# renjie-liang/HUAL

Measured on AMD Instinct MI355X. Metric: train clips/sec, higher is better.
Workload: dtype f32 (fp16x3 / bf16x3 split-operand MFMA, fp32 accumulate); 1 GPU; Charades-STA SeqPAN train step (fwd+bwd+clip+AdamWD, dropout 0.2), batch 64/GPU, T=128, vdim=1024, L=20, C=8, dim=128, 8 heads, 2 attention layers, random init; ONE batch resident in HBM, batch assembly (hual_assemble_batch) outside the timed region; global_batch=64, T=128, vdim=1024, L=20, parallelism=dp1, launch=hipGraph, video_dtype=f32

## Files before the change

hual_amd/csrc/api_kernels.cpp:

```cpp
#include "../../include/hual_seqpan.h"
#include "common.h"
#include "gemm.h"
#include "mproj.h"
#include "attn.h"
#include "heads.h"
#include "rowops.h"

namespace hual {
const char* last_error_cstr();
}

using namespace hual;

extern "C" {

int hual_abi_version(void) { return HUAL_ABI_VERSION; }
uint64_t hual_cfg_bytes(void) { return sizeof(hual_cfg); }
const char* hual_last_error(void) { return hual::last_error_cstr(); }

int hual_linear_dw(const float* A, int lda, const float* dY, int ldy, float* dW, int ldw, float* db, int M, int K,
                   int N, int workgroups, void* scratch, uint64_t scratch_bytes, void* stream) {
  HUAL_REQUIRE(A && dY && dW, "hual_linear_dw: null pointer");
  HUAL_REQUIRE(M > 0 && K % 16 == 0 && N == 128, "hual_linear_dw: K % 16 == 0 and N == 128 required");
  HUAL_REQUIRE(workgroups >= 0, "hual_linear_dw: workgroups >= 0 (0: one per CU)");
  HUAL_REQUIRE(scratch && scratch_bytes >= 4 * dw_table_words(1), "hual_linear_dw: scratch table too small");
  DwJob j;
  dw_job_init(j);
  j.npieces = 1;
  j.A[0] = A; j.lda[0] = lda; j.kw[0] = K; j.dW[0] = dW; j.ldw = ldw;
  j.dY = dY; j.ldy = ldy; j.M = M; j.N = N; j.db = db;
  DropCfg d = make_dropcfg(nullptr, 0.f);
  return launch_dw(&j, 1, d, (hipStream_t)stream, reinterpret_cast<DwJob*>(scratch), true, workgroups);
}

int hual_linear_bf16x3(const float* A, int lda, const float* W, int trans_w, const float* bias, float* Y, int ldy, int M,
                       int K, int N, int act, void* scratch, uint64_t scratch_bytes, void* stream) {
  HUAL_REQUIRE(A && W && Y && scratch, "hual_linear_bf16x3: null pointer");
  HUAL_REQUIRE(M > 0 && K > 0 && N > 0 && act >= 0 && act <= 1, "hual_linear_bf16x3: bad shape / act (0 none, 1 relu)");
  HUAL_REQUIRE((lda % 4) == 0 && (ldy % 4) == 0, "hual_linear_bf16x3: leading dims must be multiples of 4");
  const uint32_t off = 0, boff = 0;
  MProjArgs g{};
  g.R = M; g.MT = mproj_rows(M);
  if (!trans_w) {
    HUAL_REQUIRE(N == 128 && K % 8 == 0, "hual_linear_bf16x3: W must be [K,128] with K % 8 == 0");
    HUAL_REQUIRE(scratch_bytes >= (uint64_t)((K + 127) / 128) * 65536, "hual_linear_bf16x3: scratch too small (ceil(K/128) * 65536 bytes)");
// ... 92 lines not shown
```

hual_amd/csrc/dablock.h:

```cpp
#pragma once
#include "common.h"
#include "rowops.h"

namespace hual {

#define HUAL_LNPROJ_MAX 5
struct LnProjArgs {
  const float* x;
  const float* xa; int pre_site; float* x_out;
  uint8_t* pre_bits; uint8_t* y1_bits;
  const float* x2;
  const float* g1; const float* b1; float* y1;
  int drop_site1;
  const float* g2; const float* b2; float* y2;
  float* mean; float* rstd;
  int nproj;
  const float* wimg[HUAL_LNPROJ_MAX];
  const float* bias[HUAL_LNPROJ_MAX];
  float* out[HUAL_LNPROJ_MAX]; int ldo[HUAL_LNPROJ_MAX];
  int src[HUAL_LNPROJ_MAX];
  int accum[HUAL_LNPROJ_MAX];
  int act[HUAL_LNPROJ_MAX];
  int out_site[HUAL_LNPROJ_MAX];
  uint8_t* out_bits[HUAL_LNPROJ_MAX];
// ... 22 lines not shown
  int R; int MT;
  int Nv;
  uint32_t drop_row0;
};
int da_post_rows(int R, int Nv = 0);
int launch_da_post(const DaPostArgs& a, const DropCfg& drop, hipStream_t s, const LnProjArgs* tail = nullptr);

}

namespace hual {

#define HUAL_LNBWD_MAX 6
struct LnProjBwdArgs {
  int nsteps;
  const float* A[HUAL_LNBWD_MAX]; int lda[HUAL_LNBWD_MAX];
  const uint8_t* a_bits[HUAL_LNBWD_MAX];
  float* a_save[HUAL_LNBWD_MAX];
  const float* wimg_t[HUAL_LNBWD_MAX];
  int dst[HUAL_LNBWD_MAX];
  const float* add_dy1;
  const uint8_t* dy1_bits;
  const float* x; const float* mean; const float* rstd;
  const float* g1; const float* g2;
  const float* add1;
  float* dx;
  float* dz; const uint8_t* dz_bits;
  float* part;
  int R; int MT; uint32_t drop_row0;
  int Nv;
  const float* pre_x; const float* pre_mean; const float* pre_rstd; const float* pre_g; const float* pre_dy; const float* pre_add;
// ... 18 lines not shown
```

hual_amd/csrc/dablock.hip:

```cpp
#include "dablock.h"
#include "tilecore.h"
#include "prof.h"

using namespace hual;

__device__ __forceinline__ float row16_max(float v) {
  v = fmaxf(v, dpp_xor_partner(v, 1));
  v = fmaxf(v, dpp_xor_partner(v, 2));
  v = fmaxf(v, dpp_xor_partner(v, 4));
  v = fmaxf(v, dpp_xor_partner(v, 8));
  return v;
}
__device__ __forceinline__ float4 sig4(float4 v) { return make_float4(sigmoidf_(v.x), sigmoidf_(v.y), sigmoidf_(v.z), sigmoidf_(v.w)); }

#include "lnproj_body.h"

template <int NT, bool PLAIN>
__global__ __launch_bounds__(CB_THREADS) void ln_proj_kernel(LnProjArgs a, DropCfg drop) {
  extern __shared__ __attribute__((aligned(16))) char lp_lds[];
  ln_proj_body<NT, false, PLAIN>(a, drop, lp_lds);
}
template <int NT>
__global__ __launch_bounds__(CB_THREADS) void ln_proj_pair_kernel(LnProjArgs a0, LnProjArgs a1, DropCfg drop) {
  extern __shared__ __attribute__((aligned(16))) char lp_lds[];
// ... 301 lines not shown
  if (tile_ < 0) return false;
  const int r0 = tile_ * MT;
  const int RE = min(R, r0 + MT);
  const int j = lane & 15, g = lane >> 4, ecol = 16 * wave + 4 * g;
  const DropRegs dr = drop_load(drop);

  TfW w[2];
  tf_load_w(w[0], a.wimg_t[0], wave, lane);
  float4 nv[LB_U], xv[LB_U], a1v[LB_U];
  float mu[LB_U], rsd[LB_U];
  constexpr bool pre = PRE;
  const float* add1p = pre ? (a.pre_add ? a.pre_add : a.x) : (a.add1 ? a.add1 : a.x);
  const float* a0p = pre ? a.pre_dy : a.A[0];
  const int lda0 = pre ? HUAL_D : a.lda[0];
  uint32_t nkb[LB_U];
  const int nsteps = SIX ? 6 : (MID ? 1 : a.nsteps);
  auto has_bits = [&](int k) { return !SIX && a.a_bits[k] != nullptr; };
  auto to_second = [&](int k) { return SIX ? k >= 4 : a.dst[k] != 0; };
  const bool has_g2 = SIX || (!MID && a.g2 != nullptr), has_add_dy1 = SIX || (!MID && a.add_dy1 != nullptr), has_dy1_bits = !SIX && a.dy1_bits != nullptr;
  const uint8_t* kb0p = has_bits(0) ? a.a_bits[0] : reinterpret_cast<const uint8_t*>(a.x);
  float4 pxv[LB_U];
  float pmu[LB_U], prs[LB_U];
#pragma unroll
  for (int u = 0; u < LB_U; ++u) {
    const int row = min(r0 + grp + 16 * u, R - 1);
    nv[u] = ld4(a0p + (size_t)row * lda0 + col);
    nkb[u] = SIX ? 0u : kb0p[(size_t)row * 16 + (l32 >> 1)];
    xv[u] = ld4(a.x + (size_t)row * HUAL_D + col);
    a1v[u] = ld4(add1p + (size_t)row * HUAL_D + col);
    mu[u] = a.mean[row];
    rsd[u] = a.rstd[row];
    if (pre) { pxv[u] = ld4(a.pre_x + (size_t)row * HUAL_D + col); pmu[u] = a.pre_mean[row]; prs[u] = a.pre_rstd[row]; }
  }
  const float4 g1 = ld4(a.g1 + col);
  float4 sg2 = f4zero(), sb2 = f4zero();
  if (pre) {
    const float4 pg = ld4(a.pre_g + col);
#pragma unroll
    for (int u = 0; u < LB_U; ++u) {
      const int lr = grp + 16 * u;
      const bool ok = lr < MT && r0 + lr < RE;
// ... 13 lines not shown
  }
  const float4 g2 = has_g2 ? ld4(a.g2 + col) : f4zero();
  float4 addt[NT];
  const float* addp = has_add_dy1 ? a.add_dy1 : a.x;
#pragma unroll
  for (int rt = 0; rt < NT; ++rt) addt[rt] = (SIX || MID) ? f4zero() : ld4(addp + (uint32_t)min(r0 + 16 * rt + j, R - 1) * (uint32_t)HUAL_D + (uint32_t)ecol);
  auto fill = [&](int k) {
    char* S = (k & 1) ? S1 : S0;
    float* ai = (k & 1) ? ainv1 : ainv0;
#pragma unroll
    for (int u = 0; u < LB_U; ++u) {
      const int lr = grp + 16 * u, row = r0 + lr;
      if (lr >= MT) continue;
      const bool ok = row < RE;
      float4 v = ok ? nv[u] : f4zero();
      if (has_bits(k)) {
        if (dr.enabled) v = f4_select((nkb[u] >> (4 * (l32 & 1))) & 15u, make_float4(v.x * dr.scale, v.y * dr.scale, v.z * dr.scale, v.w * dr.scale));
        if (ok && a.a_save[k]) st4_nt(a.a_save[k] + (size_t)row * HUAL_D + col, v);
      }
      const float inv = cb_store_operand(S, S + LB_ROWS * 256, lr, l32, v);
      if (l32 == 0) ai[lr] = ok ? inv : 0.f;
    }
  };
  HUAL_STAMP_K(4, 0);
  fill(0);
  HUAL_STAMP_K(4, 1);
  float4 acc0[NT], acc1[NT];
  bool first0 = true, first1 = true;
#pragma unroll
  for (int rt = 0; rt < NT; ++rt) { acc0[rt] = f4zero(); acc1[rt] = f4zero(); }
#pragma unroll
  for (int k = 0; k < HUAL_LNBWD_MAX; ++k) {
    if (k >= nsteps) break;
    const bool more = k + 1 < nsteps;
    if (SIX && k == 5) {
#pragma unroll
      for (int rt = 0; rt < NT; ++rt) addt[rt] = ld4(addp + (uint32_t)min(r0 + 16 * rt + j, R - 1) * (uint32_t)HUAL_D + (uint32_t)ecol);
    }
    if (more) {
      const uint8_t* nbp = has_bits(k + 1) ? a.a_bits[k + 1] : reinterpret_cast<const uint8_t*>(a.x);
      const float* nap = a.A[k + 1];
      const int nld = a.lda[k + 1];
#pragma unroll
      for (int u = 0; u < LB_U; ++u) {
        const size_t row = (size_t)min(r0 + grp + 16 * u, R - 1);
        nv[u] = ld4(nap + row * nld + col);
        nkb[u] = SIX ? 0u : nbp[row * 16 + (l32 >> 1)];
      }
      tf_load_w(w[(k + 1) & 1], a.wimg_t[k + 1], wave, lane);
    }
// ... 452 lines not shown
    return 0;
  }
  switch (cdiv(a.MT, 16)) {
    case 1: { HUAL_DYN_LDS(da_post_kernel<1>, 160 * 1024); HUAL_LAUNCH(flops, bytes, da_post_kernel<1>, grid, dim3(CB_THREADS), lds, s, a, drop); break; }
    case 2: { HUAL_DYN_LDS(da_post_kernel<2>, 160 * 1024); HUAL_LAUNCH(flops, bytes, da_post_kernel<2>, grid, dim3(CB_THREADS), lds, s, a, drop); break; }
    default: { HUAL_DYN_LDS(da_post_kernel<3>, 160 * 1024); HUAL_LAUNCH(flops, bytes, da_post_kernel<3>, grid, dim3(CB_THREADS), lds, s, a, drop); break; }
  }
  HUAL_CHECK_HIP(hipGetLastError());
  return 0;
}

int ln_proj_bwd_rows(int R, int Nv) { return tile_rows(R, Nv, LB_ROWS); }
int ln_proj_bwd_blocks(int R, int Nv) { return cdiv(R, ln_proj_bwd_rows(R, Nv)); }

static bool ln_proj_bwd_six(const LnProjBwdArgs& a) {
  if (a.pre_x || a.nsteps != 6 || !a.g2 || !a.add_dy1 || a.dy1_bits || !a.add1) return false;
  for (int k = 0; k < 6; ++k)
    if (a.a_bits[k] || a.a_save[k] || (a.dst[k] != 0) != (k >= 4)) return false;
  return true;
}

static int check_ln_proj_bwd(const LnProjBwdArgs& a) {
  HUAL_REQUIRE(a.nsteps >= 1 && a.nsteps <= HUAL_LNBWD_MAX && a.R > 0, "ln_proj_bwd: step count / rows");
  HUAL_REQUIRE(a.MT >= 1 && a.MT <= LB_ROWS, "ln_proj_bwd: MT must be 1..48");
  HUAL_REQUIRE(a.x && a.mean && a.rstd && a.g1 && a.dx && a.part, "ln_proj_bwd: null tensor");
  bool any1 = false;
  for (int k = 0; k < a.nsteps; ++k) {
    HUAL_REQUIRE((a.A[k] || (k == 0 && a.pre_x)) && a.wimg_t[k] && (a.lda[k] % 4) == 0, "ln_proj_bwd: product operand");
    HUAL_REQUIRE(a.dst[k] == 0 || a.g2, "ln_proj_bwd: product for the absent second layer norm");
    any1 = any1 || a.dst[k] != 0;
  }
  HUAL_REQUIRE(!a.g2 || any1, "ln_proj_bwd: second layer norm without a product");
  HUAL_REQUIRE(!a.pre_x || (!a.g2 && !a.add1 && a.pre_mean && a.pre_rstd && a.pre_g && a.pre_dy), "ln_proj_bwd: layer-norm prologue");
  return 0;
}
static void ln_proj_bwd_work(const LnProjBwdArgs& a, double& flops, double& bytes) {
  const double rows = (double)a.R;
  flops += 2.0 * rows * HUAL_D * HUAL_D * a.nsteps;
  bytes += 4.0 * (rows * HUAL_D * ((a.pre_x ? 7.0 : 4.0) + a.nsteps) + (double)a.nsteps * HUAL_D * HUAL_D);
}

int launch_ln_proj_bwd(const LnProjBwdArgs& a, const DropCfg& drop, hipStream_t s) {
  int rc = check_ln_proj_bwd(a);
  if (rc) return rc;
  const size_t lds = LB_LDS;
  double flops = 0.0, bytes = 0.0;
  ln_proj_bwd_work(a, flops, bytes);
  const dim3 grid(xcd_clip_grid(a.R, a.Nv, a.MT));
  const bool six = ln_proj_bwd_six(a);
#define LN_BWD_NT(NT)                                                                                                   \
  {                                                                                                                     \
    if (a.pre_x) { HUAL_DYN_LDS((ln_proj_bwd_kernel<true, NT>), 160 * 1024); HUAL_LAUNCH(flops, bytes, (ln_proj_bwd_kernel<true, NT>), grid, dim3(CB_THREADS), lds, s, a, drop); } \
    else if (six) { HUAL_DYN_LDS((ln_proj_bwd_kernel<false, NT, true>), 160 * 1024); HUAL_LAUNCH(flops, bytes, (ln_proj_bwd_kernel<false, NT, true>), grid, dim3(CB_THREADS), lds, s, a, drop); } \
    else { HUAL_DYN_LDS((ln_proj_bwd_kernel<false, NT>), 160 * 1024); HUAL_LAUNCH(flops, bytes, (ln_proj_bwd_kernel<false, NT>), grid, dim3(CB_THREADS), lds, s, a, drop); }      \
// ... 68 lines not shown
```

hual_amd/csrc/gemm.h:

```cpp
#pragma once
#include "common.h"
#include "embed_args.h"

namespace hual {

#define HUAL_MAX_PIECES 4

struct DwJob {
  const float* A[HUAL_MAX_PIECES];
  const float* A2[HUAL_MAX_PIECES];
  int lda[HUAL_MAX_PIECES];
  int lda2[HUAL_MAX_PIECES];
  int kw[HUAL_MAX_PIECES];
  int npieces;
  int a_drop_site;
  uint32_t a_drop_row0;
  float* dW[HUAL_MAX_PIECES];
  int ldw;
  const float* dY; int ldy;
  int M, N;
  float* db;
  int a_bf16;
  const uint8_t* a_keep; int ld_keep;
};

#define HUAL_MAX_DW_JOBS 12
struct DwBatch {
  DwJob j[HUAL_MAX_DW_JOBS];
};

#define HUAL_PACK_BLOCK_BYTES (128 * 512)
struct PackExtra {
  const int32_t* lens; const int32_t* word_ids; float* rowmask; float* loss_acc; int B, T, L;
  float* zero_ptr; size_t zero_n;
  const float* E; float lambda; float* dE_ortho;
  int gather_tasks; int gather_rows; EmbedArgs emb; DropCfg drop;
  int wall_K; uint32_t wall_off, wall_boff;
  uint32_t* ovf; int novf;
// ... 30 lines not shown
```

hual_amd/csrc/gemm.hip:

```cpp
#include "gemm.h"
#include <type_traits>
#include "philox.h"
#include "bf16x3.h"
#include "tilecore.h"
#include "prof.h"
#include "ortho.h"
#include "embed_gather.h"
#include <math.h>
#include <stdlib.h>
#include <stdio.h>
#include <string.h>

namespace hual {

void dw_job_init(DwJob& j) {
  ::memset((void*)&j, 0, sizeof(j));
  j.a_drop_site = -1;
}

}

using namespace hual;

__device__ __forceinline__ float4 f4mul(float4 a, float4 b) { return make_float4(a.x * b.x, a.y * b.y, a.z * b.z, a.w * b.w); }
// ... 232 lines not shown
#define DWB_PLAIN 0
#define DWB_PROD 1
#define DWB_DROP 2
template <int MODE, int DEPTH>
__device__ __forceinline__ void dw_f16_segment(const DwJob& job, const int p, const int kb, const int m_lo, const int m_hi,
                                                const DropCfg& drop, char* ldsb, float4 (*bred)[32]) {
  const int lane = threadIdx.x & 63, wave = threadIdx.x >> 6;
  const int i = lane & 31, h = lane >> 5;
  const int kq = wave >> 2, nq = wave & 3;
  const int k0 = kb * 128;
  const int kw = job.kw[p];
  const char* Ap = reinterpret_cast<const char*>(job.A[p]);
  const char* A2p = MODE == DWB_PROD ? reinterpret_cast<const char*>(job.A2[p]) : nullptr;
  const int lda = job.lda[p], lda2 = job.lda2[p];
  const char* Yp = reinterpret_cast<const char*>(job.dY);
  const int ldy = job.ldy;
  constexpr bool PLAIN = MODE == DWB_PLAIN;
  const bool adrop = MODE == DWB_DROP && job.a_drop_site >= 0 && drop.enabled;
  const uint32_t asite = (uint32_t)job.a_drop_site;
  const uint32_t arow0 = job.a_drop_row0;
  const bool dob = (job.db != nullptr) && p == 0 && kb == 0;
  const bool abf = MODE == DWB_DROP && job.a_bf16 != 0;

  f32x16 acc[2];
#pragma unroll
  for (int c = 0; c < 2; ++c)
#pragma unroll
    for (int r = 0; r < 16; ++r) acc[c][r] = 0.f;
  float4 bsum = f4zero();
  float* mxs = reinterpret_cast<float*>(&bred[0][0]);
  float s_y = 0.f, s_y_inv = 0.f;
  float s_a = 0.f, s_a_inv = 0.f;

  const int srow = threadIdx.x >> 5, c4 = threadIdx.x & 31;
  const int kcol = k0 + 4 * c4;
  const bool kin = kcol < kw;
  const uint32_t esz = abf ? 2u : 4u;
  const uint32_t aoff = ((uint32_t)srow * (uint32_t)lda + (uint32_t)kcol) * esz;
  const uint32_t yoff = ((uint32_t)srow * (uint32_t)ldy + 4u * (uint32_t)c4) * 4u;
  struct Stage { float4 a[DWB_RU], y[DWB_RU], a2[MODE == DWB_PROD ? DWB_RU : 1]; uint32_t keep[DWB_RU]; };
  const uint32_t a2off = ((uint32_t)srow * (uint32_t)lda2 + (uint32_t)kcol) * 4u;
  const uint8_t* keepp = MODE == DWB_DROP ? job.a_keep : nullptr;
  const uint32_t koff = (uint32_t)srow * (uint32_t)job.ld_keep + (uint32_t)(kcol >> 3);
  Stage st[DEPTH - 1];
  auto stage_load = [&](int mt, Stage& st) {
    const char* Ab = Ap + (size_t)mt * lda * esz;
    const char* Yb = Yp + (size_t)mt * ldy * 4;
#pragma unroll
    for (int u = 0; u < DWB_RU; ++u) {
      const int m = mt + srow + 16 * u;
      float4 a = f4zero(), y = f4zero();
      if (m < m_hi) {
        if (kin) {
          if (abf) {
            const uint2 raw = ld2_global(Ab + 16u * u * (uint32_t)lda * 2u + aoff);
            a.x = __uint_as_float(raw.x);
            a.y = __uint_as_float(raw.y);
          } else {
            a = ld4_global(Ab + 16u * u * (uint32_t)lda * 4u + aoff);
          }
          if (MODE == DWB_PROD && A2p) st.a2[u] = ld4_global(A2p + (size_t)mt * lda2 * 4 + 16u * u * (uint32_t)lda2 * 4u + a2off);
        }
        y = ld4_global(Yb + 16u * u * (uint32_t)ldy * 4u + yoff);
        if (MODE == DWB_DROP && keepp && kin) st.keep[u] = ld1_global(keepp + (size_t)mt * job.ld_keep + 16u * u * (uint32_t)job.ld_keep + koff);
      }
      st.a[u] = a;
      st.y[u] = y;
    }
  };
  auto stage_store = [&](int buf, int mt, const Stage& st) {
    char* base = ldsb + buf * 4 * DWB_PLANE;
#pragma unroll
    for (int u = 0; u < DWB_RU; ++u) {
      const int row = srow + 16 * u;
      const int off = tile256_off(row, c4 >> 1) + 8 * (c4 & 1);
      float4 a = st.a[u];
      if (!PLAIN) {
        const int m = mt + row;
        const bool live = m < m_hi && kin;
        if (abf) {
          const uint32_t r0 = __float_as_uint(a.x), r1 = __float_as_uint(a.y);
          a = make_float4(__uint_as_float(r0 << 16), __uint_as_float(r0 & 0xffff0000u), __uint_as_float(r1 << 16),
                          __uint_as_float(r1 & 0xffff0000u));
        }
        if (MODE == DWB_PROD && A2p && live) a = f4mul(a, st.a2[u]);
        if (adrop && live) {
          a = f4mul(a, mask_from_bits4((st.keep[u] >> (4 * (c4 & 1))) & 15u, drop.scale));
        }
      }
      uint2 hi, lo;
      f16_split4_s(a, s_a, hi, lo);
      *reinterpret_cast<uint2*>(base + off) = hi;
      *reinterpret_cast<uint2*>(base + DWB_PLANE + off) = lo;
      f16_split4_s(st.y[u], s_y, hi, lo);
      *reinterpret_cast<uint2*>(base + 2 * DWB_PLANE + off) = hi;
      *reinterpret_cast<uint2*>(base + 3 * DWB_PLANE + off) = lo;
      bsum = f4add(bsum, st.y[u]);
    }
  };
  const int gq = (lane >> 2) & 3, gp = lane & 3, ghalf = (lane >> 4) & 1, gh = lane >> 5;
  auto tr_off = [&](int colbase, int ks, int rr) {
    const int row = 16 * ks + 8 * gh + 4 * rr + gq;
    const int ch = ((colbase + 16 * ghalf) >> 3) + (gp >> 1);
    return tile256_off(row, ch) + 8 * (gp & 1);
  };
  auto products = [&](int buf) {
    const char* base = ldsb + buf * 4 * DWB_PLANE;
#pragma unroll
    for (int ks = 0; ks < DWB_TM / 16; ++ks) {
      const int y0 = tr_off(nq * 32, ks, 0), y1 = tr_off(nq * 32, ks, 1);
      const f16x8 yh = join_tr_f16(lds_read_tr16(base + 2 * DWB_PLANE, y0), lds_read_tr16(base + 2 * DWB_PLANE, y1));
      const f16x8 yl = join_tr_f16(lds_read_tr16(base + 3 * DWB_PLANE, y0), lds_read_tr16(base + 3 * DWB_PLANE, y1));
// ... 4 lines not shown
        const f16x8 al = join_tr_f16(lds_read_tr16(base + DWB_PLANE, o0), lds_read_tr16(base + DWB_PLANE, o1));
        acc[c] = __builtin_amdgcn_mfma_f32_32x32x16_f16(ah, yh, acc[c], 0, 0, 0);
        acc[c] = __builtin_amdgcn_mfma_f32_32x32x16_f16(ah, yl, acc[c], 0, 0, 0);
        acc[c] = __builtin_amdgcn_mfma_f32_32x32x16_f16(al, yh, acc[c], 0, 0, 0);
      }
    }
  };

  auto put_max = [&](const Stage& st, int par) {
#ifdef DWB_EXP_FIXSCALE
    return;
#endif
    float m = 0.f, ma = 0.f;
#pragma unroll
    for (int u = 0; u < DWB_RU; ++u) {
      m = fmaxf(m, f4absmax(st.y[u]));
      float4 a = st.a[u];
      if (abf) {
        const uint32_t r0 = __float_as_uint(a.x), r1 = __float_as_uint(a.y);
        a = make_float4(__uint_as_float(r0 << 16), __uint_as_float(r0 & 0xffff0000u), __uint_as_float(r1 << 16), __uint_as_float(r1 & 0xffff0000u));
      }
      if (MODE == DWB_PROD && A2p) a = f4mul(a, st.a2[u]);
      ma = fmaxf(ma, f4absmax(a));
    }
    if (adrop) ma *= drop.scale;
    m = fast_max32(m);
    m = fmaxf(m, lane_xor32_partner(m));
    ma = fast_max32(ma);
    ma = fmaxf(ma, lane_xor32_partner(ma));
    if (lane == 0) { mxs[par * 16 + wave] = m; mxs[par * 16 + 8 + wave] = ma; }
  };
// ... 83 lines not shown
  if (dob) {
    bred[srow][c4] = bsum;
    __syncthreads();
    if (threadIdx.x < 128) {
      const int cc = threadIdx.x;
      float s = 0.f;
#pragma unroll
      for (int k = 0; k < 16; ++k) s += reinterpret_cast<const float*>(&bred[k][cc >> 2])[cc & 3];
      atomic_add_global(job.db + cc, s);
    }
  }
}

__device__ __forceinline__ void dw_f16_any_segment(const DwJob& job, const int p, const int kb, const int m_lo, const int m_hi,
                                                    const DropCfg& drop, char* ldsb, float4 (*bred)[32]) {
  if (job.A2[p]) dw_f16_segment<DWB_PROD, 2>(job, p, kb, m_lo, m_hi, drop, ldsb, bred);
  else if (job.a_bf16 || job.a_drop_site >= 0) dw_f16_segment<DWB_DROP, 4>(job, p, kb, m_lo, m_hi, drop, ldsb, bred);
  else dw_f16_segment<DWB_PLAIN, 4>(job, p, kb, m_lo, m_hi, drop, ldsb, bred);
}

#ifdef HUAL_STAMPS
#define DW_STAMP_SLOTS 16
__device__ unsigned long long g_dw_stamps[2048 * DW_STAMP_SLOTS];
extern "C" int hual_debug_dw_stamps(unsigned long long* out, int n) {
  return (int)hipMemcpyFromSymbol(out, HIP_SYMBOL(g_dw_stamps), sizeof(unsigned long long) * (size_t)n);
}
#define DW_STAMP(i, v) do { if (threadIdx.x == 0 && blockIdx.x < 2048 && (i) < DW_STAMP_SLOTS) g_dw_stamps[blockIdx.x * DW_STAMP_SLOTS + (i)] = (v); } while (0)
#else
#define DW_STAMP(i, v) do { } while (0)
#endif
#define DW_UNIT_COST 72
// ... 37 lines not shown
  DW_STAMP(5, (unsigned long long)j);
  int nseg = 0, nnp = 0;
  while (t < t_end) {
    const DwJob& job = table[j];
    const int per_unit = (job.M + DWB_TM - 1) / DWB_TM;
    const int local = t - prefix[j];
    int unit = local / per_unit;
    const int tile = local - unit * per_unit;
    const int cnt = min(per_unit - tile, t_end - t);
    int p = 0;
    for (p = 0; p < job.npieces; ++p) {
      const int nkb = (job.kw[p] + 127) >> 7;
      if (unit < nkb) break;
      unit -= nkb;
    }
    const bool plain = !job.a_bf16 && !job.A2[p] && job.a_drop_site < 0;
    dw_f16_any_segment(job, p, unit, tile * DWB_TM, min((tile + cnt) * DWB_TM, job.M), drop, reinterpret_cast<char*>(lds), bred);
    t += cnt;
    if (t >= prefix[j + 1]) ++j;
    __syncthreads();
    DW_STAMP(7 + nseg, __builtin_readcyclecounter());
    ++nseg;
    nnp += plain ? 0 : 1;
  }
  DW_STAMP(2, __builtin_readcyclecounter());
  DW_STAMP(4, (unsigned long long)nseg);
  DW_STAMP(6, (unsigned long long)nnp);
}

namespace hual {

// ... 61 lines not shown
  return 0;
}

static int dw_check(const DwJob& j, int& kbs, double& flops, double& bytes) {
  HUAL_REQUIRE(j.M > 0 && j.N == 128, "launch_dw: N must be 128");
  HUAL_REQUIRE(j.npieces >= 1 && j.npieces <= HUAL_MAX_PIECES, "launch_dw: pieces");
  kbs = 0;
  double kt = 0.0;
  for (int p = 0; p < j.npieces; ++p) {
    HUAL_REQUIRE(j.kw[p] > 0 && (j.kw[p] % 16) == 0, "launch_dw: piece width must be a multiple of 16");
    HUAL_REQUIRE(j.A[p] && j.dW[p], "launch_dw: null operand");
    HUAL_REQUIRE((j.lda[p] % 4) == 0 && (j.ldy % 4) == 0, "launch_dw: leading dims must be multiples of 4");
    kbs += cdiv(j.kw[p], 128);
    kt += j.kw[p];
  }
  flops += 2.0 * j.M * kt * j.N;
  bytes += 4.0 * ((double)j.M * kt + (double)j.M * j.N + kt * j.N);
  return 0;
}

int launch_dw(const DwJob* jobs, int n, const DropCfg& drop, hipStream_t stream, DwJob* table, bool write_table, int blocks) {
  HUAL_REQUIRE(table != nullptr && n >= 1, "launch_dw: job table");
  for (int i = 0; i < n; ++i)
    HUAL_REQUIRE(!jobs[i].a_bf16 || (jobs[i].npieces == 1 && !jobs[i].A2[0] && (jobs[i].lda[0] % 4) == 0),
                 "dw: a bfloat16 operand needs one piece, no product prologue");
  double flops = 0.0, bytes = 0.0;
  int tiles = 0, cost = 0;
  static const int wts[3] = {32, 46, 46};
  for (int base = 0; base < n; base += HUAL_MAX_DW_JOBS) {
    const int cnt = n - base < HUAL_MAX_DW_JOBS ? n - base : HUAL_MAX_DW_JOBS;
    DwBatch b;
    DwPlanPart pre;
    for (int i = 0; i < cnt; ++i) {
      const DwJob& jb = jobs[base + i];
      int kbs;
      int rc = dw_check(jb, kbs, flops, bytes);
      if (rc) return rc;
      b.j[i] = jb;
      bool prod = false;
      for (int p = 0; p < jb.npieces; ++p) prod = prod || jb.A2[p] != nullptr;
      const int w = (jb.a_drop_site >= 0 || jb.a_bf16) ? wts[2] : prod ? wts[1] : wts[0];
      pre.tiles[i] = tiles;
      pre.cost[i] = cost;
      pre.w[i] = w;
      tiles += kbs * cdiv(jb.M, DWB_TM);
      cost += kbs * (DW_UNIT_COST + cdiv(jb.M, DWB_TM) * w);
    }
    for (int i = cnt; i <= HUAL_MAX_DW_JOBS; ++i) { pre.tiles[i] = tiles; pre.cost[i] = cost; pre.w[i] = 1; }
    if (write_table) HUAL_LAUNCH(0.0, 0.0, dw_table_write_kernel, dim3(1), dim3(64), 0, stream, b, pre, table, base, cnt, n);
  }
  int dev = 0, cus = 256;
  HUAL_CHECK_HIP(hipGetDevice(&dev));
  HUAL_CHECK_HIP(hipDeviceGetAttribute(&cus, hipDeviceAttributeMultiprocessorCount, dev));
  int nblocks = blocks > 0 ? blocks : cus;
  if (nblocks > tiles) nblocks = tiles;
// ... 8 lines not shown
```

hual_amd/csrc/seqpan.hip:

```cpp
#include "attn.h"
#include "prof.h"
#include "cq.h"
#include "convblock.h"
#include "dablock.h"
#include "embed.h"
#include "gemm.h"
#include "heads.h"
#include "mproj.h"
#include "optim.h"
#include "params.h"
#include "rowops.h"
#include <stdlib.h>
#include <string.h>
#include <algorithm>
#include <unordered_map>
#include <vector>

namespace hual {
const char* last_error_cstr();
}
using namespace hual;

namespace {

// ... 1002 lines not shown
        attn_job_init(a[k]);
        a[k].Q = qkv; a[k].ldq = 3 * D; a[k].B = B; a[k].qmask = rowmask; a[k].kmask = rowmask; a[k].lddo = D; a[k].lddq = D;
        a[k].O = (k & 1) ? x_att : s_att; a[k].ldo = D;
      }
      a[0].K = qkv + D; a[0].V = qkv + 2 * D; a[0].ldkv = 3 * D; a[0].Tq = T; a[0].Tk = T; a[0].qrow0 = 0; a[0].krow0 = 0;
      a[0].dO = d_satt; a[0].dQ = dq_self; a[0].dK = d_qkv + D; a[0].dV = d_qkv + 2 * D; a[0].lddkv = 3 * D; a[0].drop_site = site + 0;
      a[1].K = ktvt; a[1].V = ktvt + D; a[1].ldkv = 2 * D; a[1].Tq = T; a[1].Tk = L; a[1].qrow0 = 0; a[1].krow0 = Nv;
      a[1].dO = d_xatt; a[1].dQ = dq_cross; a[1].dK = d_ktvt; a[1].dV = d_ktvt + D; a[1].lddkv = 2 * D; a[1].drop_site = site + 1;
      a[2].K = qkv + D; a[2].V = qkv + 2 * D; a[2].ldkv = 3 * D; a[2].Tq = L; a[2].Tk = L; a[2].qrow0 = Nv; a[2].krow0 = Nv;
      a[2].dO = d_satt; a[2].dQ = dq_self; a[2].dK = d_qkv + D; a[2].dV = d_qkv + 2 * D; a[2].lddkv = 3 * D; a[2].drop_site = site + 0;
      a[3].K = ktvt; a[3].V = ktvt + D; a[3].ldkv = 2 * D; a[3].Tq = L; a[3].Tk = T; a[3].qrow0 = Nv; a[3].krow0 = 0;
      a[3].dO = d_xatt; a[3].dQ = dq_cross; a[3].dK = d_ktvt; a[3].dV = d_ktvt + D; a[3].lddkv = 2 * D; a[3].drop_site = site + 1;
      for (int k = 0; k < 4; ++k) set_dmask(c, a[k], t + ".dm" + std::to_string(k));
      c.attn_bwd(a, 4);
    }
    c.push_dw(mkdw(ln1, D, D, dq_self, D, R, c.g(d.query.k), c.g(d.query.b)));
    c.push_dw(mkdw(ln1, D, D, dq_cross, D, R, c.g(d.query.k), c.g(d.query.b)));
    c.push_dw(mkdw(ln1, D, D, d_qkv + D, 3 * D, R, c.g(d.f_key.k), c.g(d.f_key.b)));
    c.push_dw(mkdw(ln1, D, D, d_qkv + 2 * D, 3 * D, R, c.g(d.f_value.k), c.g(d.f_value.b)));
    c.push_dw(mkdw(lnt, D, D, d_ktvt, 2 * D, R, c.g(d.t_key.k), c.g(d.t_key.b)));
    c.push_dw(mkdw(lnt, D, D, d_ktvt + D, 2 * D, R, c.g(d.t_value.k), c.g(d.t_value.b)));
    float* d_xin = c.act(dt + ".in");
    float* nz = nullptr; const uint8_t* nz_bits = nullptr;
    if (li > 0) { nz = c.act("d.da" + std::to_string(li - 1) + ".z2"); nz_bits = c.bits("da" + std::to_string(li - 1) + ".kb4", R); }
    {
      LnProjBwdArgs lb{};
      lb.nsteps = 6;
      const float* As[6] = {dq_self, dq_cross, d_qkv + D, d_qkv + 2 * D, d_ktvt, d_ktvt + D};
      const int lds_[6] = {D, D, 3 * D, 3 * D, 2 * D, 2 * D};
      const size_t wo[6] = {d.query.k, d.query.k, d.f_key.k, d.f_value.k, d.t_key.k, d.t_value.k};
      for (int k = 0; k < 6; ++k) { lb.A[k] = As[k]; lb.lda[k] = lds_[k]; lb.wimg_t[k] = imgt(wo[k]); lb.dst[k] = k < 4 ? 0 : 1; }
      lb.add_dy1 = d_ln1a; lb.x = xin; lb.mean = mean; lb.rstd = rstd; lb.g1 = c.p(d.ln1.g); lb.g2 = c.p(d.lnt.g);
      lb.add1 = d_res; lb.dx = d_xin; lb.dz = nz; lb.dz_bits = nz_bits; lb.R = R; lb.Nv = Nv; lb.drop_row0 = 0;
      c.ln_proj_bwd(lb, c.g(d.ln1.g), c.g(d.ln1.b), c.g(d.lnt.g), c.g(d.lnt.b));
    }
    dx = d_xin;
  }
  float* x0 = c.act("cb.x0");
  c.stage(ST_CONV);
  float* d_x0 = conv_block_bwd(c, "cb", x0, dx, pm.cb, c.rs, HUAL_SITE_CONV);
  c.stage(ST_ALWAYS);
  PosBwdJob pj[2];
  int npj = 0;
  if (!c.dry && c.stage_on(ST_INPUT)) pj[npj++] = PosBwdJob{{d_x0, nullptr}, c.g(pm.pos), 1, 1};
  if (!c.dry && c.stage_on(ST_PRED)) pj[npj++] = PosBwdJob{{fe_dx0[1], fe_dx0[0]}, c.g(pm.fe_pos), 1, 0};
  const bool pos_rides = c.sel_stage < 0;
// ... 393 lines not shown
```

hual_amd/lib.py:

```python
import ctypes
import os

_HERE = os.path.dirname(os.path.abspath(__file__))
LIB_PATH = os.environ.get('HUAL_LIB_PATH') or os.path.join(_HERE, 'libhual_seqpan.so')
ABI_VERSION = 9

_lib = None


class HualError(RuntimeError):
    pass


class hual_cfg(ctypes.Structure):
    _fields_ = [('vdim', ctypes.c_int32), ('dim', ctypes.c_int32), ('num_heads', ctypes.c_int32),
                ('word_dim', ctypes.c_int32), ('char_dim', ctypes.c_int32), ('max_vlen', ctypes.c_int32),
                ('attn_layer', ctypes.c_int32), ('num_chars', ctypes.c_int32), ('num_words', ctypes.c_int32),
                ('no_gumbel', ctypes.c_int32), ('match_lambda', ctypes.c_float), ('tau', ctypes.c_float),
                ('clip_norm', ctypes.c_float), ('finetune_word_emb', ctypes.c_int32)]


class hual_param_entry(ctypes.Structure):
    _fields_ = [('name', ctypes.c_char * 112), ('offset', ctypes.c_uint64), ('size', ctypes.c_uint64),
                ('ndim', ctypes.c_int32), ('shape', ctypes.c_int32 * 4), ('decay', ctypes.c_int32)]
# ... 92 lines not shown
    lib.hual_predictor_fwd.argtypes = blk + [vp, vp, vp, vp, vp, vp, u64, vp]
    lib.hual_predictor_bwd.argtypes = blk + [vp, vp, vp, vp, vp, u64, vp]
    lib.hual_prof_get.argtypes = [i32, ctypes.c_char_p, i32, P(ctypes.c_int64), P(ctypes.c_double), P(ctypes.c_double),
                                  P(ctypes.c_double)]
    lib.hual_prof_kernel_pipe.argtypes = [ctypes.c_char_p, P(i32), P(i32)]
    lib.hual_linear_bf16x3.argtypes = [vp, i32, vp, i32, vp, vp, i32, i32, i32, i32, i32, vp, u64, vp]
    lib.hual_layer_norm_fwd.argtypes = [vp, vp, vp, vp, vp, vp, i32, vp]
    lib.hual_attention_fwd.argtypes = [vp, i32, vp, vp, i32, vp, i32, i32, i32, i32, vp, vp, vp]
    lib.hual_attention_fwd_save.argtypes = [vp, i32, vp, vp, i32, vp, i32, i32, i32, i32, vp, vp, vp, vp, i32, vp, f32, i32, vp]
    lib.hual_attention_bwd.argtypes = [vp, i32, vp, vp, i32, vp, i32, vp, vp, i32, vp, i32, vp, i32, vp, vp, i32, i32, i32, i32, vp, vp,
                                       vp, f32, i32, vp]
    lib.hual_attention_keep_row_bytes.argtypes = [i32]
    lib.hual_span_argmax.argtypes = [vp, vp, vp, vp, vp, i32, i32, vp]
    lib.hual_span_topk.argtypes = [vp, vp, vp, i32, i32, i32, i32, f32, vp, vp, vp, vp]
    lib.hual_linear_dw.argtypes = [vp, i32, vp, i32, vp, i32, vp, i32, i32, i32, i32, vp, u64, vp]
    lib.hual_al_score.argtypes = [P(hual_al_set), vp, vp, vp, vp, vp, vp, f32, vp, vp, vp, vp, vp, vp]
    lib.hual_al_renew.argtypes = [P(hual_al_set), vp, i32, vp, vp, vp, P(ctypes.c_double), vp, vp]
    lib.hual_assemble_batch.argtypes = [P(hual_dataset), vp, i32, i32, i32, i32, vp, vp, vp, vp, vp, vp, vp, vp, vp]
    lib.hual_assemble_batch_carry.argtypes = [P(hual_dataset), vp, i32, i32, i32, i32, vp, vp, vp, vp, vp, vp, vp, vp, vp, vp, i32, vp]
    _lib = lib
    return lib


def check(code):
    if code != 0:
        raise HualError('libhual_seqpan: %s (code %d)' % (load().hual_last_error().decode(), code))


def ptr(t):
    return None if t is None else ctypes.c_void_p(t.data_ptr())
# ... 66 lines not shown
    return {e.name.decode(): (int(e.offset), int(e.rows), int(e.cols)) for e in arr}


def linear_bf16x3(A, W, bias=None, act=0, trans_w=False):
    import torch
    M, K = A.shape
    N = W.shape[0] if trans_w else W.shape[1]
    Y = torch.empty(M, N, device=A.device, dtype=torch.float32)
    nbytes = ((N + 127) // 128) * 65536 if trans_w else ((K + 127) // 128) * 65536
    scratch = torch.zeros(nbytes, dtype=torch.uint8, device=A.device)
    check(load().hual_linear_bf16x3(ptr(A), A.stride(0), ptr(W), int(trans_w), ptr(bias), ptr(Y), Y.stride(0), M, K, N, act,
                                    ptr(scratch), nbytes, stream_ptr()))
    return Y


def linear_dw(A, dY, dW, db=None, workgroups=0):
    M, K = A.shape
    N = dY.shape[1]
    import torch
    scratch = torch.empty(256, dtype=torch.float32, device=A.device)
    check(load().hual_linear_dw(ptr(A), A.stride(0), ptr(dY), dY.stride(0), ptr(dW), dW.stride(0), ptr(db), M, K, N,
                                workgroups, ptr(scratch), 1024, stream_ptr()))


def span_topk(start_logits, end_logits, video_seq_len, k, max_len=0, nms_iou=1.0, out=None):
    import torch
    if start_logits.dtype != torch.float32 or end_logits.dtype != torch.float32:
        raise HualError('span_topk: float32 logits required')
    if start_logits.dim() != 2 or end_logits.shape != start_logits.shape:
        raise HualError('span_topk: start / end logits must both be [B,T]')
    s, e = start_logits.contiguous(), end_logits.contiguous()
    B, T = s.shape
    vl = video_seq_len.to(device=s.device, dtype=torch.int32).contiguous()
    if vl.numel() != B:
        raise HualError('span_topk: video_seq_len must hold B = %d lengths' % B)
    k = int(k)
    if out is None:
# ... 10 lines not shown
```

include/hual_seqpan.h:

```cpp
#ifndef HUAL_SEQPAN_H
#define HUAL_SEQPAN_H

#include <stddef.h>
#include <stdint.h>

#ifdef __cplusplus
extern "C" {
#endif

#define HUAL_ABI_VERSION 9

#define HUAL_OK 0
#define HUAL_ERR_INVALID (-1)
#define HUAL_ERR_HIP (-2)
#define HUAL_ERR_UNSUPPORTED (-3)
#define HUAL_ERR_WORKSPACE (-4)

#define HUAL_SITE_WORD 0
#define HUAL_SITE_CHAR 1
#define HUAL_SITE_VIDEO 2
#define HUAL_SITE_CONV 3
#define HUAL_SITE_DA 8
#define HUAL_SITE_TRI 24
#define HUAL_SITE_GUMBEL 28
// ... 135 lines not shown
                     float* feats, void* workspace, uint64_t ws_bytes, void* stream);
int hual_cq_attn_bwd(const hual_cfg* cfg, const float* params, const hual_batch* batch, const hual_run_opts* opts, const float* dfeats,
                     float* dx, float* grads, void* workspace, uint64_t ws_bytes, void* stream);
int hual_predictor_fwd(const hual_cfg* cfg, const float* params, const hual_batch* batch, const hual_run_opts* opts, const float* outputs,
                       float* start_logits, float* end_logits, int64_t* start_index, int64_t* end_index, void* workspace,
                       uint64_t ws_bytes, void* stream);
int hual_predictor_bwd(const hual_cfg* cfg, const float* params, const hual_batch* batch, const hual_run_opts* opts, const float* d_start,
                       const float* d_end, float* d_outputs, float* grads, void* workspace, uint64_t ws_bytes, void* stream);


int hual_linear_bf16x3(const float* A, int lda, const float* W, int trans_w, const float* bias, float* Y, int ldy, int M,
                       int K, int N, int act, void* scratch, uint64_t scratch_bytes, void* stream);

int hual_linear_dw(const float* A, int lda, const float* dY, int ldy, float* dW, int ldw, float* db, int M, int K,
                   int N, int workgroups, void* scratch, uint64_t scratch_bytes, void* stream);

int hual_layer_norm_fwd(const float* x, const float* gamma, const float* beta, float* y, float* mean, float* rstd, int R,
                        void* stream);

int hual_attention_fwd(const float* Q, int ldq, const float* K, const float* V, int ldkv, float* O, int ldo, int B, int Tq,
                       int Tk, const float* qmask, const float* kmask, void* stream);

int hual_attention_fwd_save(const float* Q, int ldq, const float* K, const float* V, int ldkv, float* O, int ldo, int B, int Tq,
                            int Tk, const float* qmask, const float* kmask, float* stats, uint8_t* keep_bytes, int ldm,
                            const uint32_t* rng_state, float drop_rate, int drop_site, void* stream);
int hual_attention_keep_row_bytes(int Tk);

int hual_attention_bwd(const float* Q, int ldq, const float* K, const float* V, int ldkv, const float* O, int ldo,
                       const float* stats, const uint8_t* keep_bytes, int ldm, const float* dO, int lddo, float* dQ, int lddq,
                       float* dK, float* dV, int lddkv, int B, int Tq, int Tk, const float* qmask, const float* kmask,
// ... 62 lines not shown
```

Measured before the change: 53660 clips/s.

## Sum self and cross query gradients before shared-weight dW and input-gradient GEMMs

```diff
diff --git a/hual_amd/csrc/api_kernels.cpp b/hual_amd/csrc/api_kernels.cpp
--- a/hual_amd/csrc/api_kernels.cpp
+++ b/hual_amd/csrc/api_kernels.cpp
@@ -20,6 +20,11 @@
 
 int hual_linear_dw(const float* A, int lda, const float* dY, int ldy, float* dW, int ldw, float* db, int M, int K,
                    int N, int workgroups, void* scratch, uint64_t scratch_bytes, void* stream) {
+  return hual_linear_dw_sum(A, lda, dY, nullptr, ldy, dW, ldw, db, M, K, N, workgroups, scratch, scratch_bytes, stream);
+}
+
+int hual_linear_dw_sum(const float* A, int lda, const float* dY, const float* dY2, int ldy, float* dW, int ldw, float* db, int M,
+                       int K, int N, int workgroups, void* scratch, uint64_t scratch_bytes, void* stream) {
   HUAL_REQUIRE(A && dY && dW, "hual_linear_dw: null pointer");
   HUAL_REQUIRE(M > 0 && K % 16 == 0 && N == 128, "hual_linear_dw: K % 16 == 0 and N == 128 required");
   HUAL_REQUIRE(workgroups >= 0, "hual_linear_dw: workgroups >= 0 (0: one per CU)");
@@ -28,7 +33,7 @@
   dw_job_init(j);
   j.npieces = 1;
   j.A[0] = A; j.lda[0] = lda; j.kw[0] = K; j.dW[0] = dW; j.ldw = ldw;
-  j.dY = dY; j.ldy = ldy; j.M = M; j.N = N; j.db = db;
+  j.dY = dY; j.dY2 = dY2; j.ldy = ldy; j.M = M; j.N = N; j.db = db;
   DropCfg d = make_dropcfg(nullptr, 0.f);
   return launch_dw(&j, 1, d, (hipStream_t)stream, reinterpret_cast<DwJob*>(scratch), true, workgroups);
 }
diff --git a/hual_amd/csrc/dablock.h b/hual_amd/csrc/dablock.h
--- a/hual_amd/csrc/dablock.h
+++ b/hual_amd/csrc/dablock.h
@@ -60,6 +60,7 @@
 struct LnProjBwdArgs {
   int nsteps;
   const float* A[HUAL_LNBWD_MAX]; int lda[HUAL_LNBWD_MAX];
+  const float* A2[HUAL_LNBWD_MAX];
   const uint8_t* a_bits[HUAL_LNBWD_MAX];
   float* a_save[HUAL_LNBWD_MAX];
   const float* wimg_t[HUAL_LNBWD_MAX];
diff --git a/hual_amd/csrc/dablock.hip b/hual_amd/csrc/dablock.hip
--- a/hual_amd/csrc/dablock.hip
+++ b/hual_amd/csrc/dablock.hip
@@ -339,9 +339,10 @@
   const float* a0p = pre ? a.pre_dy : a.A[0];
   const int lda0 = pre ? HUAL_D : a.lda[0];
   uint32_t nkb[LB_U];
-  const int nsteps = SIX ? 6 : (MID ? 1 : a.nsteps);
+  float4 nv2[LB_U];
+  const int nsteps = SIX ? 5 : (MID ? 1 : a.nsteps);
   auto has_bits = [&](int k) { return !SIX && a.a_bits[k] != nullptr; };
-  auto to_second = [&](int k) { return SIX ? k >= 4 : a.dst[k] != 0; };
+  auto to_second = [&](int k) { return SIX ? k >= 3 : a.dst[k] != 0; };
   const bool has_g2 = SIX || (!MID && a.g2 != nullptr), has_add_dy1 = SIX || (!MID && a.add_dy1 != nullptr), has_dy1_bits = !SIX && a.dy1_bits != nullptr;
   const uint8_t* kb0p = has_bits(0) ? a.a_bits[0] : reinterpret_cast<const uint8_t*>(a.x);
   float4 pxv[LB_U];
@@ -350,6 +351,7 @@
   for (int u = 0; u < LB_U; ++u) {
     const int row = min(r0 + grp + 16 * u, R - 1);
     nv[u] = ld4(a0p + (size_t)row * lda0 + col);
+    if (SIX) nv2[u] = ld4(a.A2[0] + (size_t)row * lda0 + col);
     nkb[u] = SIX ? 0u : kb0p[(size_t)row * 16 + (l32 >> 1)];
     xv[u] = ld4(a.x + (size_t)row * HUAL_D + col);
     a1v[u] = ld4(add1p + (size_t)row * HUAL_D + col);
@@ -393,6 +395,7 @@
       if (lr >= MT) continue;
       const bool ok = row < RE;
       float4 v = ok ? nv[u] : f4zero();
+      if (SIX && k == 0 && ok) v = make_float4(__fadd_rn(v.x, nv2[u].x), __fadd_rn(v.y, nv2[u].y), __fadd_rn(v.z, nv2[u].z), __fadd_rn(v.w, nv2[u].w));
       if (has_bits(k)) {
         if (dr.enabled) v = f4_select((nkb[u] >> (4 * (l32 & 1))) & 15u, make_float4(v.x * dr.scale, v.y * dr.scale, v.z * dr.scale, v.w * dr.scale));
         if (ok && a.a_save[k]) st4_nt(a.a_save[k] + (size_t)row * HUAL_D + col, v);
@@ -412,7 +415,7 @@
   for (int k = 0; k < HUAL_LNBWD_MAX; ++k) {
     if (k >= nsteps) break;
     const bool more = k + 1 < nsteps;
-    if (SIX && k == 5) {
+    if (SIX && k == 4) {
 #pragma unroll
       for (int rt = 0; rt < NT; ++rt) addt[rt] = ld4(addp + (uint32_t)min(r0 + 16 * rt + j, R - 1) * (uint32_t)HUAL_D + (uint32_t)ecol);
     }
@@ -895,9 +898,9 @@
 int ln_proj_bwd_blocks(int R, int Nv) { return cdiv(R, ln_proj_bwd_rows(R, Nv)); }
 
 static bool ln_proj_bwd_six(const LnProjBwdArgs& a) {
-  if (a.pre_x || a.nsteps != 6 || !a.g2 || !a.add_dy1 || a.dy1_bits || !a.add1) return false;
-  for (int k = 0; k < 6; ++k)
-    if (a.a_bits[k] || a.a_save[k] || (a.dst[k] != 0) != (k >= 4)) return false;
+  if (a.pre_x || a.nsteps != 5 || !a.A2[0] || !a.g2 || !a.add_dy1 || a.dy1_bits || !a.add1) return false;
+  for (int k = 0; k < 5; ++k)
+    if (a.a_bits[k] || a.a_save[k] || (a.dst[k] != 0) != (k >= 3)) return false;
   return true;
 }
 
@@ -912,13 +915,17 @@
     any1 = any1 || a.dst[k] != 0;
   }
   HUAL_REQUIRE(!a.g2 || any1, "ln_proj_bwd: second layer norm without a product");
+  for (int k = 0; k < a.nsteps; ++k)
+    HUAL_REQUIRE(!a.A2[k] || (k == 0 && ln_proj_bwd_six(a)), "ln_proj_bwd: a summed operand (A2) is the first product of the dual attention's shape");
   HUAL_REQUIRE(!a.pre_x || (!a.g2 && !a.add1 && a.pre_mean && a.pre_rstd && a.pre_g && a.pre_dy), "ln_proj_bwd: layer-norm prologue");
   return 0;
 }
 static void ln_proj_bwd_work(const LnProjBwdArgs& a, double& flops, double& bytes) {
   const double rows = (double)a.R;
   flops += 2.0 * rows * HUAL_D * HUAL_D * a.nsteps;
-  bytes += 4.0 * (rows * HUAL_D * ((a.pre_x ? 7.0 : 4.0) + a.nsteps) + (double)a.nsteps * HUAL_D * HUAL_D);
+  int nops = a.nsteps;
+  for (int k = 0; k < a.nsteps; ++k) nops += a.A2[k] ? 1 : 0;
+  bytes += 4.0 * (rows * HUAL_D * ((a.pre_x ? 7.0 : 4.0) + nops) + (double)a.nsteps * HUAL_D * HUAL_D);
 }
 
 int launch_ln_proj_bwd(const LnProjBwdArgs& a, const DropCfg& drop, hipStream_t s) {
diff --git a/hual_amd/csrc/gemm.h b/hual_amd/csrc/gemm.h
--- a/hual_amd/csrc/gemm.h
+++ b/hual_amd/csrc/gemm.h
@@ -22,6 +22,7 @@
   float* db;
   int a_bf16;
   const uint8_t* a_keep; int ld_keep;
+  const float* dY2;
 };
 
 #define HUAL_MAX_DW_JOBS 12
diff --git a/hual_amd/csrc/gemm.hip b/hual_amd/csrc/gemm.hip
--- a/hual_amd/csrc/gemm.hip
+++ b/hual_amd/csrc/gemm.hip
@@ -270,6 +270,7 @@
   const char* A2p = MODE == DWB_PROD ? reinterpret_cast<const char*>(job.A2[p]) : nullptr;
   const int lda = job.lda[p], lda2 = job.lda2[p];
   const char* Yp = reinterpret_cast<const char*>(job.dY);
+  const char* Y2p = MODE == DWB_PROD ? reinterpret_cast<const char*>(job.dY2) : nullptr;
   const int ldy = job.ldy;
   constexpr bool PLAIN = MODE == DWB_PLAIN;
   const bool adrop = MODE == DWB_DROP && job.a_drop_site >= 0 && drop.enabled;
@@ -294,7 +295,8 @@
   const uint32_t esz = abf ? 2u : 4u;
   const uint32_t aoff = ((uint32_t)srow * (uint32_t)lda + (uint32_t)kcol) * esz;
   const uint32_t yoff = ((uint32_t)srow * (uint32_t)ldy + 4u * (uint32_t)c4) * 4u;
-  struct Stage { float4 a[DWB_RU], y[DWB_RU], a2[MODE == DWB_PROD ? DWB_RU : 1]; uint32_t keep[DWB_RU]; };
+  struct Stage { float4 a[DWB_RU], y[DWB_RU], a2[MODE == DWB_PROD ? DWB_RU : 1], y2[MODE == DWB_PROD ? DWB_RU : 1]; uint32_t keep[DWB_RU]; };
+  auto ysum = [&](const Stage& st, int u) { return (MODE == DWB_PROD && Y2p) ? f4add(st.y[u], st.y2[u]) : st.y[u]; };
   const uint32_t a2off = ((uint32_t)srow * (uint32_t)lda2 + (uint32_t)kcol) * 4u;
   const uint8_t* keepp = MODE == DWB_DROP ? job.a_keep : nullptr;
   const uint32_t koff = (uint32_t)srow * (uint32_t)job.ld_keep + (uint32_t)(kcol >> 3);
@@ -318,8 +320,10 @@
           if (MODE == DWB_PROD && A2p) st.a2[u] = ld4_global(A2p + (size_t)mt * lda2 * 4 + 16u * u * (uint32_t)lda2 * 4u + a2off);
         }
         y = ld4_global(Yb + 16u * u * (uint32_t)ldy * 4u + yoff);
+        if (MODE == DWB_PROD && Y2p) st.y2[u] = ld4_global(Y2p + (size_t)mt * ldy * 4 + 16u * u * (uint32_t)ldy * 4u + yoff);
         if (MODE == DWB_DROP && keepp && kin) st.keep[u] = ld1_global(keepp + (size_t)mt * job.ld_keep + 16u * u * (uint32_t)job.ld_keep + koff);
       }
+      else if (MODE == DWB_PROD && Y2p) st.y2[u] = f4zero();
       st.a[u] = a;
       st.y[u] = y;
     }
@@ -348,10 +352,11 @@
       f16_split4_s(a, s_a, hi, lo);
       *reinterpret_cast<uint2*>(base + off) = hi;
       *reinterpret_cast<uint2*>(base + DWB_PLANE + off) = lo;
-      f16_split4_s(st.y[u], s_y, hi, lo);
+      const float4 y = ysum(st, u);
+      f16_split4_s(y, s_y, hi, lo);
       *reinterpret_cast<uint2*>(base + 2 * DWB_PLANE + off) = hi;
       *reinterpret_cast<uint2*>(base + 3 * DWB_PLANE + off) = lo;
-      bsum = f4add(bsum, st.y[u]);
+      bsum = f4add(bsum, y);
     }
   };
   const int gq = (lane >> 2) & 3, gp = lane & 3, ghalf = (lane >> 4) & 1, gh = lane >> 5;
@@ -386,7 +391,7 @@
     float m = 0.f, ma = 0.f;
 #pragma unroll
     for (int u = 0; u < DWB_RU; ++u) {
-      m = fmaxf(m, f4absmax(st.y[u]));
+      m = fmaxf(m, f4absmax(ysum(st, u)));
       float4 a = st.a[u];
       if (abf) {
         const uint32_t r0 = __float_as_uint(a.x), r1 = __float_as_uint(a.y);
@@ -500,7 +505,7 @@
 
 __device__ __forceinline__ void dw_f16_any_segment(const DwJob& job, const int p, const int kb, const int m_lo, const int m_hi,
                                                     const DropCfg& drop, char* ldsb, float4 (*bred)[32]) {
-  if (job.A2[p]) dw_f16_segment<DWB_PROD, 2>(job, p, kb, m_lo, m_hi, drop, ldsb, bred);
+  if (job.A2[p] || job.dY2) dw_f16_segment<DWB_PROD, 2>(job, p, kb, m_lo, m_hi, drop, ldsb, bred);
   else if (job.a_bf16 || job.a_drop_site >= 0) dw_f16_segment<DWB_DROP, 4>(job, p, kb, m_lo, m_hi, drop, ldsb, bred);
   else dw_f16_segment<DWB_PLAIN, 4>(job, p, kb, m_lo, m_hi, drop, ldsb, bred);
 }
@@ -568,7 +573,7 @@
       if (unit < nkb) break;
       unit -= nkb;
     }
-    const bool plain = !job.a_bf16 && !job.A2[p] && job.a_drop_site < 0;
+    const bool plain = !job.a_bf16 && !job.A2[p] && !job.dY2 && job.a_drop_site < 0;
     dw_f16_any_segment(job, p, unit, tile * DWB_TM, min((tile + cnt) * DWB_TM, job.M), drop, reinterpret_cast<char*>(lds), bred);
     t += cnt;
     if (t >= prefix[j + 1]) ++j;
@@ -660,8 +665,9 @@
     kbs += cdiv(j.kw[p], 128);
     kt += j.kw[p];
   }
+  HUAL_REQUIRE(!j.dY2 || (!j.a_bf16 && j.a_drop_site < 0), "launch_dw: a summed gradient (dY2) goes with plain or product operands");
   flops += 2.0 * j.M * kt * j.N;
-  bytes += 4.0 * ((double)j.M * kt + (double)j.M * j.N + kt * j.N);
+  bytes += 4.0 * ((double)j.M * kt + (double)j.M * j.N * (j.dY2 ? 2.0 : 1.0) + kt * j.N);
   return 0;
 }
 
@@ -685,6 +691,7 @@
       b.j[i] = jb;
       bool prod = false;
       for (int p = 0; p < jb.npieces; ++p) prod = prod || jb.A2[p] != nullptr;
+      prod = prod || jb.dY2 != nullptr;
       const int w = (jb.a_drop_site >= 0 || jb.a_bf16) ? wts[2] : prod ? wts[1] : wts[0];
       pre.tiles[i] = tiles;
       pre.cost[i] = cost;
diff --git a/hual_amd/csrc/seqpan.hip b/hual_amd/csrc/seqpan.hip
--- a/hual_amd/csrc/seqpan.hip
+++ b/hual_amd/csrc/seqpan.hip
@@ -1040,8 +1040,16 @@
       for (int k = 0; k < 4; ++k) set_dmask(c, a[k], t + ".dm" + std::to_string(k));
       c.attn_bwd(a, 4);
     }
+#ifndef HUAL_QSUM_TWO_DW_JOBS
+    {
+      DwJob j = mkdw(ln1, D, D, dq_self, D, R, c.g(d.query.k), c.g(d.query.b));
+      j.dY2 = dq_cross;
+      c.push_dw(j);
+    }
+#else
     c.push_dw(mkdw(ln1, D, D, dq_self, D, R, c.g(d.query.k), c.g(d.query.b)));
     c.push_dw(mkdw(ln1, D, D, dq_cross, D, R, c.g(d.query.k), c.g(d.query.b)));
+#endif
     c.push_dw(mkdw(ln1, D, D, d_qkv + D, 3 * D, R, c.g(d.f_key.k), c.g(d.f_key.b)));
     c.push_dw(mkdw(ln1, D, D, d_qkv + 2 * D, 3 * D, R, c.g(d.f_value.k), c.g(d.f_value.b)));
     c.push_dw(mkdw(lnt, D, D, d_ktvt, 2 * D, R, c.g(d.t_key.k), c.g(d.t_key.b)));
@@ -1051,11 +1059,12 @@
     if (li > 0) { nz = c.act("d.da" + std::to_string(li - 1) + ".z2"); nz_bits = c.bits("da" + std::to_string(li - 1) + ".kb4", R); }
     {
       LnProjBwdArgs lb{};
-      lb.nsteps = 6;
-      const float* As[6] = {dq_self, dq_cross, d_qkv + D, d_qkv + 2 * D, d_ktvt, d_ktvt + D};
-      const int lds_[6] = {D, D, 3 * D, 3 * D, 2 * D, 2 * D};
-      const size_t wo[6] = {d.query.k, d.query.k, d.f_key.k, d.f_value.k, d.t_key.k, d.t_value.k};
-      for (int k = 0; k < 6; ++k) { lb.A[k] = As[k]; lb.lda[k] = lds_[k]; lb.wimg_t[k] = imgt(wo[k]); lb.dst[k] = k < 4 ? 0 : 1; }
+      lb.nsteps = 5;
+      const float* As[5] = {dq_self, d_qkv + D, d_qkv + 2 * D, d_ktvt, d_ktvt + D};
+      const int lds_[5] = {D, 3 * D, 3 * D, 2 * D, 2 * D};
+      const size_t wo[5] = {d.query.k, d.f_key.k, d.f_value.k, d.t_key.k, d.t_value.k};
+      for (int k = 0; k < 5; ++k) { lb.A[k] = As[k]; lb.lda[k] = lds_[k]; lb.wimg_t[k] = imgt(wo[k]); lb.dst[k] = k < 3 ? 0 : 1; }
+      lb.A2[0] = dq_cross;
       lb.add_dy1 = d_ln1a; lb.x = xin; lb.mean = mean; lb.rstd = rstd; lb.g1 = c.p(d.ln1.g); lb.g2 = c.p(d.lnt.g);
       lb.add1 = d_res; lb.dx = d_xin; lb.dz = nz; lb.dz_bits = nz_bits; lb.R = R; lb.Nv = Nv; lb.drop_row0 = 0;
       c.ln_proj_bwd(lb, c.g(d.ln1.g), c.g(d.ln1.b), c.g(d.lnt.g), c.g(d.lnt.b));
diff --git a/hual_amd/lib.py b/hual_amd/lib.py
--- a/hual_amd/lib.py
+++ b/hual_amd/lib.py
@@ -130,6 +130,7 @@
     lib.hual_span_argmax.argtypes = [vp, vp, vp, vp, vp, i32, i32, vp]
     lib.hual_span_topk.argtypes = [vp, vp, vp, i32, i32, i32, i32, f32, vp, vp, vp, vp]
     lib.hual_linear_dw.argtypes = [vp, i32, vp, i32, vp, i32, vp, i32, i32, i32, i32, vp, u64, vp]
+    lib.hual_linear_dw_sum.argtypes = [vp, i32, vp, vp, i32, vp, i32, vp, i32, i32, i32, i32, vp, u64, vp]
     lib.hual_al_score.argtypes = [P(hual_al_set), vp, vp, vp, vp, vp, vp, f32, vp, vp, vp, vp, vp, vp]
     lib.hual_al_renew.argtypes = [P(hual_al_set), vp, i32, vp, vp, vp, P(ctypes.c_double), vp, vp]
     lib.hual_assemble_batch.argtypes = [P(hual_dataset), vp, i32, i32, i32, i32, vp, vp, vp, vp, vp, vp, vp, vp, vp]
@@ -226,13 +227,15 @@
     return Y
 
 
-def linear_dw(A, dY, dW, db=None, workgroups=0):
+def linear_dw(A, dY, dW, db=None, workgroups=0, dY2=None):
     M, K = A.shape
     N = dY.shape[1]
     import torch
+    if dY2 is not None and (dY2.shape != dY.shape or dY2.stride(0) != dY.stride(0)):
+        raise HualError('linear_dw: dY2 must have the shape and row stride of dY')
     scratch = torch.empty(256, dtype=torch.float32, device=A.device)
-    check(load().hual_linear_dw(ptr(A), A.stride(0), ptr(dY), dY.stride(0), ptr(dW), dW.stride(0), ptr(db), M, K, N,
-                                workgroups, ptr(scratch), 1024, stream_ptr()))
+    check(load().hual_linear_dw_sum(ptr(A), A.stride(0), ptr(dY), ptr(dY2), dY.stride(0), ptr(dW), dW.stride(0), ptr(db), M, K, N,
+                                    workgroups, ptr(scratch), 1024, stream_ptr()))
 
 
 def span_topk(start_logits, end_logits, video_seq_len, k, max_len=0, nms_iou=1.0, out=None):
diff --git a/include/hual_seqpan.h b/include/hual_seqpan.h
--- a/include/hual_seqpan.h
+++ b/include/hual_seqpan.h
@@ -173,6 +173,8 @@
 
 int hual_linear_dw(const float* A, int lda, const float* dY, int ldy, float* dW, int ldw, float* db, int M, int K,
                    int N, int workgroups, void* scratch, uint64_t scratch_bytes, void* stream);
+int hual_linear_dw_sum(const float* A, int lda, const float* dY, const float* dY2, int ldy, float* dW, int ldw, float* db, int M,
+                       int K, int N, int workgroups, void* scratch, uint64_t scratch_bytes, void* stream);
 
 int hual_layer_norm_fwd(const float* x, const float* gamma, const float* beta, float* y, float* mean, float* rstd, int R,
                         void* stream);
```

After: 53650 clips/s. About the same (-0.0%).
